# ACMEAtronOmatic/DSen2

Hardware: AMD Instinct MI355X
Metric: 32x32x6 patches/sec (DSen2_20, d=6, batch 512) (higher is better)
Workload: dtype f32; 1 GPU; DSen2_20 d=6 F=128 fp32, 512 synthetic 32x32 patches (4+6 bands) per GPU per step, he_uniform random-init weights; batch_per_gpu=512, parallelism=patch-sharded dp1, backend=rccl, output_gather=False

## Files before the change

### dsen2_amd/DSen2Net.py

```python
import ctypes
import sys
import threading

import numpy as np
import torch

from . import _lib, weights as _weights

RES_SCALE = 0.1
PRECISIONS = {'fp32': 0, 'bf16': 1, 'bf16x3': 2}


def _ptr(t):
    return ctypes.c_void_p(t.data_ptr()) if t is not None else ctypes.c_void_p(0)


def _stream_ptr(device):
    return ctypes.c_void_p(torch.cuda.current_stream(device).cuda_stream)


class S2Model(object):

    def __init__(self, input_shape, num_layers, feature_size, device=None, precision='fp32'):
        if len(input_shape) not in (2, 3):
# ... 96 lines not shown

    def profile_forward(self, xs, out=None, iters=10, warm=3):
        n, _, h, w = xs[0].shape
        out = self._check_out(out, n, h, w)
        ws = self._get_workspace(self.workspace_bytes(n, h, w))
        ms = (ctypes.c_float * 5)()
        with torch.cuda.device(self.device):
            _lib.call('dsen2_model_forward_profile', self._handle, _ptr(xs[0]), _ptr(xs[1]),
                      _ptr(xs[2]) if len(xs) == 3 else ctypes.c_void_p(0), _ptr(out), n, h, w,
                      _ptr(ws), ws.numel(), _stream_ptr(self.device), int(warm), int(iters), ms)
        return dict(forward_ms=ms[0], first_ms=ms[1], body_ms=ms[2], out_ms=ms[3], wall_ms=ms[4])

    def body_launches(self, n, h, w):
        with torch.cuda.device(self.device):
            r = _lib.load().dsen2_model_body_launches(self._handle, int(n), int(h), int(w))
        if r < 0:
            raise _lib.DSen2Error(r, _lib.load().dsen2_last_error().decode())
        return r

    def batch_limit(self, h, w):
        per = self.workspace_bytes(1, h, w)
        return max(1, int(self.max_workspace_bytes // per))

    def preferred_batch(self, h, w):
        limit = self.batch_limit(h, w)
        if self.precision == 'fp32' or self.num_layers <= 0:
            return limit
        cus = int(torch.cuda.get_device_properties(self.device).multi_processor_count)
        n = (limit // cus) * cus
        while n >= cus:
# ... 339 lines not shown
    xb = to_blocked(x_bf16)
    out = None
    if epilogue == 0:
        out = torch.empty((n, feat // 8, h, w, 8), dtype=torch.bfloat16, device=x_bf16.device)
    elif epilogue == 3:
        out = torch.empty((n, h, w, feat), dtype=torch.float32, device=x_bf16.device)
    with torch.cuda.device(x_bf16.device):
        _lib.call('dsen2_conv3x3_body_bf16', _ptr(xb), kernel_hwio.ctypes.data_as(_lib.c_float_p),
                  bias.ctypes.data_as(_lib.c_float_p), _ptr(res_hi), _ptr(res_lo), _ptr(out), n, h, w, feat, int(epilogue),
                  float(res_scale), _stream_ptr(x_bf16.device))
    if epilogue == 1:
        return res_hi, res_lo
    return from_blocked(out) if epilogue == 0 else out


def conv3x3_nhwc(x, kernel_hwio, bias, epilogue=0, aux=None, res_scale=RES_SCALE, ref=False):
    n, h, w, cin = x.shape
    kernel_hwio = np.ascontiguousarray(kernel_hwio, np.float32)
    bias = np.ascontiguousarray(bias, np.float32)
    cout = kernel_hwio.shape[3]
    if epilogue == 2:
        out = torch.empty((n, cout, h, w), dtype=torch.float32, device=x.device)
    else:
        out = torch.empty((n, h, w, cout), dtype=torch.float32, device=x.device)
    with torch.cuda.device(x.device):
        _lib.call('dsen2_conv3x3_nhwc_ref' if ref else 'dsen2_conv3x3_nhwc', _ptr(x), kernel_hwio.ctypes.data_as(_lib.c_float_p),
                  bias.ctypes.data_as(_lib.c_float_p), _ptr(aux), _ptr(out), n, h, w, cin, cout, int(epilogue),
                  float(res_scale), _stream_ptr(x.device))
    return out
```

### dsen2_amd/_lib.py

```python
import ctypes
import os
import sys

_HERE = os.path.dirname(os.path.abspath(__file__))
LIB_PATH = os.environ.get('DSEN2_HIP_LIB') or os.path.join(_HERE, 'libdsen2_hip.so')

OK = 0
ERR_INVALID, ERR_HIP, ERR_NO_WEIGHTS, ERR_WORKSPACE, ERR_NO_DEVICE, ERR_NOMEM, ERR_INTERNAL = -1, -2, -3, -4, -5, -6, -7
DTYPE_U16, DTYPE_F32 = 0, 1
DTYPE_F64 = 2

c_float_p = ctypes.POINTER(ctypes.c_float)
c_int_p = ctypes.POINTER(ctypes.c_int)
c_void_p = ctypes.c_void_p
c_int = ctypes.c_int
c_size_t = ctypes.c_size_t

SIGNATURES = {
    'dsen2_version': (ctypes.c_char_p, []),
    'dsen2_last_error': (ctypes.c_char_p, []),
    'dsen2_device_count': (c_int, []),
    'dsen2_model_create': (c_int, [ctypes.POINTER(c_void_p), c_int, c_int, c_int, c_int, c_int, c_int]),
    'dsen2_model_destroy': (None, [c_void_p]),
    'dsen2_model_num_params': (c_size_t, [c_void_p]),
    'dsen2_model_load_weights': (c_int, [c_void_p, c_float_p, c_size_t]),
    'dsen2_model_workspace_bytes': (c_int, [c_void_p, c_int, c_int, c_int, ctypes.POINTER(c_size_t)]),
    'dsen2_model_forward': (c_int, [c_void_p, c_void_p, c_void_p, c_void_p, c_void_p, c_int, c_int, c_int,
                                    c_void_p, c_size_t, c_void_p]),
    'dsen2_model_body_launches': (c_int, [c_void_p, c_int, c_int, c_int]),
    'dsen2_model_forward_timed': (c_int, [c_void_p, c_void_p, c_void_p, c_void_p, c_void_p, c_int, c_int, c_int,
                                          c_void_p, c_size_t, c_void_p, c_int, c_float_p]),
    'dsen2_model_forward_profile': (c_int, [c_void_p, c_void_p, c_void_p, c_void_p, c_void_p, c_int, c_int, c_int,
                                            c_void_p, c_size_t, c_void_p, c_int, c_int, c_float_p]),
    'dsen2_conv3x3_nhwc': (c_int, [c_void_p, c_float_p, c_float_p, c_void_p, c_void_p, c_int, c_int, c_int, c_int,
                                   c_int, c_int, ctypes.c_float, c_void_p]),
    'dsen2_conv3x3_nhwc_ref': (c_int, [c_void_p, c_float_p, c_float_p, c_void_p, c_void_p, c_int, c_int, c_int, c_int,
                                       c_int, c_int, ctypes.c_float, c_void_p]),
    'dsen2_split_f32': (c_int, [c_void_p, c_void_p, c_void_p, c_int, c_int, c_int, c_int, c_void_p]),
    'dsen2_join_f32': (c_int, [c_void_p, c_void_p, c_void_p, c_int, c_int, c_int, c_int, c_void_p]),
    'dsen2_conv3x3_body_bf16': (c_int, [c_void_p, c_float_p, c_float_p, c_void_p, c_void_p, c_void_p, c_int, c_int, c_int,
                                        c_int, c_int, ctypes.c_float, c_void_p]),
    'dsen2_conv3x3_first_planes': (c_int, [c_void_p, c_void_p, c_void_p, c_int, c_int, c_int, c_float_p, c_float_p, c_int, c_int,
                                           c_void_p, c_void_p, c_int, c_int, c_int, c_void_p]),
    'dsen2_split3_f32': (c_int, [c_void_p, c_void_p, c_void_p, c_int, c_int, c_int, c_int, c_void_p]),
    'dsen2_conv3x3_body_bf16x3': (c_int, [c_void_p, c_float_p, c_float_p, c_void_p, c_void_p, c_void_p, c_int, c_int, c_int,
                                          c_int, c_int, ctypes.c_float, c_void_p]),
    'dsen2_model_time_body_conv': (c_int, [c_void_p, c_int, c_void_p, c_void_p, c_void_p, c_int, c_int, c_int, c_int,
                                           c_void_p, c_float_p]),
    'dsen2_model_train_workspace_bytes': (c_int, [c_void_p, c_int, c_int, c_int, ctypes.POINTER(c_size_t)]),
    'dsen2_model_gradients': (c_int, [c_void_p, c_void_p, c_void_p, c_void_p, c_void_p, c_void_p, c_void_p, c_void_p, c_int,
                                      c_int, c_int, c_void_p, c_size_t, c_void_p]),
    'dsen2_model_get_weights': (c_int, [c_void_p, c_void_p, c_void_p]),
# ... 75 lines not shown
```

### dsen2_amd/build.py

```python
import concurrent.futures
import os
import subprocess
import sys
import tempfile

HERE = os.path.dirname(os.path.abspath(__file__))
CSRC = os.path.join(HERE, 'csrc')
SOURCES = ['conv3x3_body32.hip', 'conv3x3_body16w.hip', 'conv3x3_out.hip', 'conv3x3_out_mfma.hip', 'conv3x3_mfma.hip', 'conv3x3_first.hip', 'conv3x3_first16.hip', 'patch_ops.hip', 'down_pixel_aggr.hip', 'imresize.hip', 'conv_plan.hip', 'capi.hip',
           'conv3x3_wgrad.hip', 'train_ops.hip', 'capi_train.hip']
HEADERS = [os.path.join(CSRC, "dsen2_internal.h"), os.path.join(CSRC, "conv_plan.h"), os.path.join(CSRC, "capi_internal.h"), os.path.join(CSRC, "conv3x3_dma.h"), os.path.join(CSRC, "conv3x3_bf16_common.h"), os.path.join(os.path.dirname(HERE), 'include', 'dsen2_hip.h')]
LIB = os.path.join(HERE, 'libdsen2_hip.so')
DIAG_LIB = os.path.join(os.path.dirname(HERE), 'build', 'libdsen2_hip_diag.so')
HIPCC = os.environ.get('HIPCC', '/opt/rocm/bin/hipcc')
FLAGS = ['--offload-arch=gfx950', '-O3', '-std=c++17', '-fPIC', '-fno-gpu-rdc', '-ffp-contract=off',
         '-Wall', '-Wno-unused-function', '-Werror=array-bounds']
JOBS = int(os.environ.get('DSEN2_BUILD_JOBS', '4'))


def needs_build(lib=LIB):
    if not os.path.exists(lib):
        return True
    t = os.path.getmtime(lib)
    deps = [os.path.join(CSRC, s) for s in SOURCES] + HEADERS + [os.path.abspath(__file__),
                                                                os.path.join(HERE, 'asm_contract.py')]
# ... 41 lines not shown
```

### dsen2_amd/csrc/capi.hip

```cpp

#include <chrono>
#include <cstdarg>
#include <cstdio>
#include <cstring>
#include <exception>
#include <new>
#include <vector>

#include "capi_internal.h"

using namespace dsen2;

namespace {

thread_local char g_err[512] = "";

#ifdef DSEN2_DIAG
Tuning g_diag_tuning;
unsigned long long* g_diag_stamps = nullptr;
#endif
Tuning default_tuning() {
#ifdef DSEN2_DIAG
  return g_diag_tuning;
#else
// ... 94 lines not shown
    return p;
  };
  r.x0 = take(align_up(pix * 16));
  r.a = take(full);
  if (m->precision == 1) {
    r.hi = take(half); r.lo = take(half); r.tbf = take(half);
  } else if (m->precision == 2) {
    r.hx = take(full); r.lo16 = take(half); r.t2 = take(full);
  } else {
    r.t = take(full);
  }
  r.bytes = off * sizeof(float);
  return r;
}

int forward_launches(const dsen2_model* m, const float* x10, const float* x20, const float* x60, float* out, int n, int h, int w,
                     const ForwardWs& B, size_t keep_step, bool x0_packed, hipStream_t stream, const hipEvent_t* ev) {
  const float* P = m->dev_params;
  const int d = m->num_layers;
  if (ev) HIP_TRY(hipEventRecord(ev[0], stream));
  if (int rc = first_layer(m, x10, x20, x60, n, h, w, B, x0_packed, stream)) return rc;
  if (ev) HIP_TRY(hipEventRecord(ev[1], stream));
  if (m->precision == 2 && d > 0) {
    if (int rc = body16(m, B.hx, B.lo16, B.t2, B.a, n, h, w, stream)) return rc;
  } else if (m->precision == 1 && d > 0) {
    if (int rc = body16(m, B.hi, B.lo, B.tbf, B.a, n, h, w, stream)) return rc;
  } else {
    for (int l = 1; l <= d; ++l) {
      const Layer& LA = m->layers[2 * l - 1];
      const Layer& LB = m->layers[2 * l];
      const float* x_in = B.a + (size_t)(l - 1) * keep_step;
      float* t = B.t + (size_t)(l - 1) * keep_step;
      HIP_TRY(launch(LA.plan, make_params(x_in, LA.weights(P), LA.bias(P), nullptr, t, n, h, w, 0, 0.f), LA.plan.epilogue, m->tune, stream));
      HIP_TRY(launch(LB.plan, make_params(t, LB.weights(P), LB.bias(P), x_in, B.a + (size_t)l * keep_step, n, h, w, 0, 0.1f),
                     LB.plan.epilogue, m->tune, stream));
    }
  }
  if (ev) HIP_TRY(hipEventRecord(ev[2], stream));
  {
    const Layer& L = m->layers.back();
    const float* skip = m->c60 > 0 ? x60 : x20;
// ... 50 lines not shown
    HIP_TRY(hipEventElapsedTime(&v, e[1], e[2])); sum[2] += v;
    HIP_TRY(hipEventElapsedTime(&v, e[2], e[3])); sum[3] += v;
  }
  for (int k = 0; k < 4; ++k) ms[k] = (float)(sum[k] / iters);
  double wall = std::chrono::duration<double, std::milli>(t1 - t0).count();
  if (warm > 0) {
    float span = 0.f;
    HIP_TRY(hipEventElapsedTime(&span, evs.ev.front(), evs.ev.back()));
    wall = span;
  }
  ms[4] = (float)(wall / iters);
  return DSEN2_OK;
}

static int conv3x3_nhwc(const float* dev_in, const float* host_kernel, const float* host_bias, const float* dev_aux, float* dev_out,
                        int n, int h, int w, int cin, int cout, int epilogue, float res_scale, void* stream_, const Tuning& tune) {
  if (!dev_in || !host_kernel || !host_bias || !dev_out) return fail(DSEN2_ERR_INVALID, "NULL argument");
  if (epilogue != kEpiRelu && epilogue != kEpiResidual && epilogue != kEpiSkipNCHW) return fail(DSEN2_ERR_INVALID, "epilogue %d", epilogue);
  if (epilogue != kEpiRelu && !dev_aux) return fail(DSEN2_ERR_INVALID, "epilogue %d needs dev_aux", epilogue);
  if (int rc = check_shape(nullptr, n, h, w)) return rc;
  const ConvRole role = epilogue == kEpiSkipNCHW ? ConvRole::Output
                        : cin <= 16 ? (epilogue == kEpiRelu ? ConvRole::First : ConvRole::DgradOutput)
                        : epilogue == kEpiRelu ? ConvRole::BodyA : ConvRole::BodyB;
  ConvPlan pl;
  if (!plan_conv(role, cin, cout, 0, tune, nullptr, &pl) || pl.cin_pad != cin)
    return fail(DSEN2_ERR_INVALID, "unsupported conv %d->%d epilogue %d", cin, cout, epilogue);
  hipStream_t stream = (hipStream_t)stream_;
  std::vector<float> staged(pl.floats);
  pack(pl, host_kernel, host_bias, staged.data());
  return launch_once_with_temp("conv3x3", staged.data(), staged.size() * sizeof(float), stream, [&](char* dev) {
    const float* wpk = reinterpret_cast<const float*>(dev);
    return launch(pl, make_params(dev_in, wpk, wpk + pl.bias_off, dev_aux, dev_out, n, h, w, cout, res_scale), epilogue, tune, stream);
  });
}

static int conv3x3_body16(int precision, const void* dev_in, const float* host_kernel, const float* host_bias, void* s0, void* s1,
                          void* dev_out, int n, int h, int w, int feat, int epilogue, float res_scale, void* stream_) {
  const bool x3 = precision == 2;
  if (!dev_in || !host_kernel || !host_bias) return fail(DSEN2_ERR_INVALID, "NULL argument");
  if (feat != 128 && feat != 256) return fail(DSEN2_ERR_INVALID, "feat %d unsupported", feat);
  if (epilogue != kEpiRelu && epilogue != kEpiResidual && epilogue != kEpiResidualF32) return fail(DSEN2_ERR_INVALID, "epilogue %d", epilogue);
  if (epilogue != kEpiRelu && (!s0 || !s1))
    return fail(DSEN2_ERR_INVALID, x3 ? "residual epilogue needs the stream's tensors" : "residual epilogue needs the hi and lo planes");
  if (epilogue != kEpiResidual && !dev_out) return fail(DSEN2_ERR_INVALID, "dev_out is NULL");
  if (int rc = check_shape(nullptr, n, h, w)) return rc;
  hipStream_t stream = (hipStream_t)stream_;
  const Tuning tune = default_tuning();
// ... 43 lines not shown

const char* dsen2_version(void) {
#ifdef DSEN2_DIAG
  return "dsen2_hip 0.3-diag (gfx950; fp32 MFMA 32x32x2 / bf16 MFMA 16x16x32 / bf16x3; DIAGNOSTIC build)";
#else
  return "dsen2_hip 0.3 (gfx950; fp32 MFMA 32x32x2 / bf16 MFMA 16x16x32 / bf16x3)";
#endif
}
const char* dsen2_last_error(void) { return g_err; }

#ifdef DSEN2_DIAG
int dsen2_diag_set(int key, int value) {
  Tuning& t = g_diag_tuning;
  switch (key) {
    case 0:
      if (value != 0 && (value < 11 || value > 14)) return fail(DSEN2_ERR_INVALID, "body variant %d unknown", value);
      t.first = value == 0 ? FirstKernel::Tile16 : FirstKernel::Direct;
      t.body = value == 0 ? BodyKernel::Tile : BodyKernel::Body32;
      t.body32 = value == 0 ? Body32Form::DeferStagger : static_cast<Body32Form>(value - 11);
      return DSEN2_OK;
    case 2:
      if (value != 0 && value != 2 && value != 3) return fail(DSEN2_ERR_INVALID, "output variant %d unknown", value);
      t.out = value == 2 ? OutKernel::MfmaThenValu : value == 3 ? OutKernel::Valu : OutKernel::Tile;
      return DSEN2_OK;
    case 1: t.ablate = value; return DSEN2_OK;
    case 3: t.grid_cap = value; return DSEN2_OK;
    case 4: t.chain = value; return DSEN2_OK;
    case 5: t.first_ablate = value; return DSEN2_OK;
    case 6: t.out_ablate = value; return DSEN2_OK;
  }
  return fail(DSEN2_ERR_INVALID, "unknown diagnostic key %d", key);
// ... 26 lines not shown
    if (c10 <= 0 || c20 <= 0 || c60 < 0 || num_layers < 0) return fail(DSEN2_ERR_INVALID, "bad channel/layer counts");
    if (feature_size != 128 && feature_size != 256)
      return fail(DSEN2_ERR_INVALID, "feature_size %d unsupported (128 or 256)", feature_size);
    if (precision < 0 || precision > 2)
      return fail(DSEN2_ERR_INVALID, "precision %d unknown (0 = fp32, 1 = bf16 operands, 2 = bf16x3)", precision);
    const int cin = c10 + c20 + c60;
    const int cout = c60 > 0 ? c60 : c20;
    if (cin > 16) return fail(DSEN2_ERR_INVALID, "%d input channels > 16", cin);
    if (cout > 32) return fail(DSEN2_ERR_INVALID, "%d output channels > 32", cout);
    dsen2_model* m = new (std::nothrow) dsen2_model();
    if (!m) return fail(DSEN2_ERR_INVALID, "out of host memory");
    m->c10 = c10; m->c20 = c20; m->c60 = c60; m->cin = cin; m->cout = cout;
    m->num_layers = num_layers; m->feat = feature_size; m->precision = precision;
    m->dev_params = nullptr; m->loaded = false; m->train = nullptr;
    m->tune = default_tuning();
    if (hipGetDevice(&m->device) != hipSuccess) {
      delete m;
      return fail(DSEN2_ERR_NO_DEVICE, "no HIP device");
    }
    if (!plan_network(c10, c20, c60, num_layers, feature_size, precision, m->tune, m)) {
      delete m;
      return fail(DSEN2_ERR_INVALID, "no kernel for a layer of this network");
    }
    *out = m;
    return DSEN2_OK;
  });
}

void dsen2_model_destroy(dsen2_model* m) {
  if (!m) return;
  train_state_destroy(m->train);
  if (m->dev_params) (void)hipFree(m->dev_params);
  delete m;
}

size_t dsen2_model_num_params(const dsen2_model* m) { return m ? m->n_params : 0; }

int dsen2_model_load_weights(dsen2_model* m, const float* host_flat, size_t count) {
  return guarded([&]() -> int {
    if (!m || !host_flat) return fail(DSEN2_ERR_INVALID, "NULL argument");
    if (count != m->n_params)
      return fail(DSEN2_ERR_INVALID, "expected %zu parameters, got %zu", m->n_params, count);
    if (int rc = check_device(m)) return rc;
    std::vector<float> staged(m->dev_param_floats);
    for (const Layer& L : m->layers) {
      const float* k = host_flat + L.flat_off;
// ... 18 lines not shown
  return guarded([&] { return forward(m, x10, x20, x60, out, n, h, w, workspace, workspace_bytes, stream, nullptr); });
}

int dsen2_model_body_launches(const dsen2_model* m, int n, int h, int w) {
  return guarded([&]() -> int {
    if (!m) return fail(DSEN2_ERR_INVALID, "NULL model");
    if (int rc = check_shape(m, n, h, w)) return rc;
    if (int rc = check_device(m)) return rc;
    int dev = 0, cus = 0;
    if (hipGetDevice(&dev) != hipSuccess || hipDeviceGetAttribute(&cus, hipDeviceAttributeMultiprocessorCount, dev) != hipSuccess)
      return fail(DSEN2_ERR_NO_DEVICE, "no HIP device");
    return may_chain(m) && body16w_chain_patches_per_wg(n, h, w, m->feat, cus) > 0 ? 1 : 2 * m->num_layers;
  });
}

int dsen2_model_forward_timed(dsen2_model* m, const float* x10, const float* x20, const float* x60, float* out, int n, int h, int w,
                              void* workspace, size_t workspace_bytes, void* stream, int iters, float* body_ms_per_launch) {
  return guarded([&]() -> int {
    if (!body_ms_per_launch) return fail(DSEN2_ERR_INVALID, "NULL result");
    if (!m || m->num_layers <= 0) return fail(DSEN2_ERR_INVALID, "model has no residual blocks");
    float ms[5];
    int rc = forward_profile(m, x10, x20, x60, out, n, h, w, workspace, workspace_bytes, stream, 0, iters, ms);
    if (rc == DSEN2_OK) *body_ms_per_launch = ms[2] / (2.0f * m->num_layers);
    return rc;
  });
}

int dsen2_model_forward_profile(dsen2_model* m, const float* x10, const float* x20, const float* x60, float* out, int n, int h,
                                int w, void* workspace, size_t workspace_bytes, void* stream, int warm, int iters, float* ms5) {
  return guarded([&] { return forward_profile(m, x10, x20, x60, out, n, h, w, workspace, workspace_bytes, stream, warm, iters, ms5); });
}

int dsen2_conv3x3_nhwc(const float* dev_in, const float* host_kernel, const float* host_bias, const float* dev_aux, float* dev_out,
                       int n, int h, int w, int cin, int cout, int epilogue, float res_scale, void* stream) {
  return guarded([&] {
    return conv3x3_nhwc(dev_in, host_kernel, host_bias, dev_aux, dev_out, n, h, w, cin, cout, epilogue, res_scale, stream, default_tuning());
  });
}

int dsen2_conv3x3_nhwc_ref(const float* dev_in, const float* host_kernel, const float* host_bias, const float* dev_aux,
                           float* dev_out, int n, int h, int w, int cin, int cout, int epilogue, float res_scale, void* stream) {
  return guarded([&] {
    return conv3x3_nhwc(dev_in, host_kernel, host_bias, dev_aux, dev_out, n, h, w, cin, cout, epilogue, res_scale, stream,
                        Tuning::reference());
  });
}

int dsen2_split_f32(const float* dev_in, void* dev_hi, void* dev_lo, int n, int h, int w, int c, void* stream) {
  return guarded([&]() -> int {
    if (int rc = check_split_args(dev_in, dev_hi, dev_lo, n, h, w, c)) return rc;
    if (n == 0) return DSEN2_OK;
// ... 139 lines not shown
```

### dsen2_amd/csrc/capi_internal.h

```cpp
#pragma once
#include <exception>
#include <new>
#include <vector>

#include "../../include/dsen2_hip.h"
#include "conv_plan.h"

namespace dsen2 {

int fail(int code, const char* fmt, ...);

#define HIP_TRY(expr)                                                                                              \
  do {                                                                                                             \
    hipError_t e_ = (expr);                                                                                        \
    if (e_ != hipSuccess) return dsen2::fail(DSEN2_ERR_HIP, "%s failed: %s", #expr, hipGetErrorString(e_));   \
  } while (0)

template <class F>
int guarded(F&& body) noexcept {
  try {
    return body();
  } catch (const std::bad_alloc&) {
    return fail(DSEN2_ERR_NOMEM, "out of host memory");
  } catch (const std::exception& e) {
// ... 4 lines not shown
}

struct TrainState;
void train_state_destroy(TrainState* t);
int train_state_after_load(dsen2_model* m);

}

struct dsen2_model : dsen2::NetworkPlan {
  int c10, c20, c60, cin, cout, num_layers, feat, precision;
  int device;
  dsen2::Tuning tune;
  float* dev_params;
  bool loaded;
  dsen2::TrainState* train;
};

namespace dsen2 {

inline int check_shape(const dsen2_model* m, int n, int h, int w) {
  if (n <= 0 || h <= 0 || w <= 0) return fail(DSEN2_ERR_INVALID, "bad shape n=%d h=%d w=%d", n, h, w);
  if ((size_t)h * w * (size_t)(m ? m->feat : 256) >= ((size_t)1 << 29))
    return fail(DSEN2_ERR_INVALID, "one image of %dx%d exceeds 2^31 activation bytes", h, w);
  return DSEN2_OK;
}

inline int check_device(const dsen2_model* m) {
  int dev = -1;
  if (hipGetDevice(&dev) != hipSuccess) return fail(DSEN2_ERR_NO_DEVICE, "no HIP device");
  if (dev != m->device)
// ... 42 lines not shown
  if (e != hipSuccess) return fail(DSEN2_ERR_HIP, "%s launch: %s", what, hipGetErrorString(e));
  return DSEN2_OK;
}

struct ForwardWs {
  float* x0 = nullptr;
  float* a = nullptr;
  float* t = nullptr;
  void *hi = nullptr, *lo = nullptr, *tbf = nullptr;
  void *hx = nullptr, *lo16 = nullptr, *t2 = nullptr;
  size_t bytes = 0;
};
ForwardWs forward_ws(const dsen2_model* m, int n, int h, int w, char* base);
int forward_launches(const dsen2_model* m, const float* x10, const float* x20, const float* x60, float* out, int n, int h, int w,
                     const ForwardWs& B, size_t keep_step, bool x0_packed, hipStream_t stream, const hipEvent_t* ev);

}
```

### dsen2_amd/csrc/conv3x3_body32.hip

```cpp
#include <type_traits>

#include "conv3x3_dma.h"

namespace dsen2 {

namespace {

typedef float f32x4 __attribute__((ext_vector_type(4)));
typedef float f32x16 __attribute__((ext_vector_type(16)));
typedef unsigned u32x4 __attribute__((ext_vector_type(4)));

using dma::KC; using dma::NT; using dma::THREADS; using dma::QS; using dma::IN_BYTES; using dma::IN_BLOCKS;
using dma::WCH; using dma::NWBUF; using dma::LDS_BYTES; using dma::wait_vmcnt;
constexpr int KSTEPS = 4;
constexpr int PB = 2, MB = 2;
static_assert((8 * kHalo) % 16 == 0, "rows R and R+8 of a pixel block sit on the same banks");

}

template <int CIN, int COUT, int EPI, int ABL, int PRE, bool STG, bool DEFER>
__global__ __launch_bounds__(THREADS, 2) void conv3x3_body32_kernel(const ConvParams p, const int n_items) {
  constexpr int NCC = CIN / KC;
  constexpr int NS = COUT / NT;
  static_assert(NCC % 2 == 0, "input double buffer parity");
// ... 255 lines not shown
  auto kern = conv3x3_body32_kernel<CIN, COUT, EPI, ABL, PRE, STG, DEFER>;
  static KernelOnce once;
  int cus = 0;
  hipError_t e = once.prepare(reinterpret_cast<const void*>(kern), LDS_BYTES, &cus);
  if (e != hipSuccess) return e;
  const long long items = (long long)p.n * p.tiles_x * p.tiles_y * (COUT / NT);
  if (items <= 0 || items > 0x7fffffffLL) return hipErrorInvalidValue;
  const int grid = (int)(items < cus ? items : cus);
  hipLaunchKernelGGL(kern, dim3(grid), dim3(THREADS), LDS_BYTES, stream, p, (int)items);
  return hipGetLastError();
}

template <int F>
static hipError_t launch_body32_feat(const ConvParams& p, int epilogue, Body32Form form, hipStream_t stream) {
  const bool relu = epilogue == kEpiRelu;
#ifdef DSEN2_DIAG
  if (form == Body32Form::Plain || form == Body32Form::StaggerA) {
    if (!relu) return launch_body32_one<F, F, kEpiResidual, 0, 2, false>(p, stream);
    return form == Body32Form::Plain ? launch_body32_one<F, F, kEpiRelu, 0, 0, false>(p, stream) : launch_body32_one<F, F, kEpiRelu, 0, 0, true>(p, stream);
  }
  if (form == Body32Form::DeferStaggerA && !relu) return launch_body32_one<F, F, kEpiResidual, 0, 0, false, true>(p, stream);
#else
  if (form != Body32Form::DeferStagger) return hipErrorInvalidValue;
#endif
  return relu ? launch_body32_one<F, F, kEpiRelu, 0, 0, true, true>(p, stream) : launch_body32_one<F, F, kEpiResidual, 0, 0, true, true>(p, stream);
}

hipError_t launch_conv3x3_body32(const ConvParams& p, int feat, int epilogue, Body32Form form, int ablate, hipStream_t stream) {
  if ((size_t)p.h * p.w * feat * 4 >= 0x80000000ull) return hipErrorNotSupported;
#ifdef DSEN2_DIAG
// ... 18 lines not shown
```

### dsen2_amd/csrc/conv_plan.h

```cpp
#pragma once
#include <vector>

#include "dsen2_internal.h"

namespace dsen2 {

enum class ConvRole { First, BodyA, BodyB, Output, DgradBody, DgradOutput };
enum class ConvKernel {
  Tile,
  Body32,
  Body16,
  Body16x3,
  Out
};

constexpr size_t kAlignFloats = 64;
inline size_t align_up(size_t v) { return (v + kAlignFloats - 1) / kAlignFloats * kAlignFloats; }

struct ConvPlan {
  ConvRole role;
  ConvKernel kernel;
  int epilogue;
  int cin, cout;
  int cin_pad, cout_pad;
// ... 1 lines not shown
  int real_channels;
  Body32Form body32;
  bool out_mfma;
  bool first_direct;
  int first16_planes;
  size_t weight_floats, bias_off, first16_off, floats;
};

struct BandGroups { int c10, c20, c60; };
bool plan_conv(ConvRole role, int cin, int cout, int precision, const Tuning& tune, const BandGroups* bands, ConvPlan* plan);
void pack(const ConvPlan& plan, const float* kernel_hwio, const float* bias, float* dst);
hipError_t launch(const ConvPlan& plan, const ConvParams& p, int epilogue, const Tuning& tune, hipStream_t stream);

inline hipError_t try_launch(hipError_t e, bool* done) { *done = e == hipSuccess; return e == hipErrorNotSupported ? hipSuccess : e; }

struct Layer {
  ConvPlan plan;
  size_t off, flat_off;
  const float* weights(const float* params) const { return params + off; }
  const float* bias(const float* params) const { return params + off + plan.bias_off; }
  const float* first16(const float* params) const { return params + off + plan.first16_off; }
};
struct NetworkPlan {
  std::vector<Layer> layers;
  size_t n_params = 0;
  size_t dev_param_floats = 0;
  size_t chain_stride = 0;
};
bool plan_network(int c10, int c20, int c60, int num_layers, int feat, int precision, const Tuning& tune, NetworkPlan* net);

// ... 2 lines not shown
```

### dsen2_amd/csrc/conv_plan.hip

```cpp
#include <cstring>
#include <vector>

#include "conv_plan.h"

namespace dsen2 {

namespace {

constexpr int kBody16Chunk = 32;

bool sentinel2(const BandGroups* b) { return b && b->c10 == 4 && b->c20 == 6 && (b->c60 == 0 || b->c60 == 2); }

void pack_tile_weights(const float* k, const ConvPlan& pl, float* dst) {
  const int ncc = pl.cin_pad / pl.kc, nslab = pl.cout_pad / pl.nt, ng = pl.kc / 4;
  size_t i = 0;
  for (int slab = 0; slab < nslab; ++slab)
    for (int cc = 0; cc < ncc; ++cc)
      for (int tap = 0; tap < 9; ++tap)
        for (int gg = 0; gg < ng; ++gg)
          for (int o = 0; o < pl.nt; ++o)
            for (int j = 0; j < 4; ++j, ++i) {
              const int c = cc * pl.kc + 4 * gg + j, oc = slab * pl.nt + o;
              dst[i] = (c < pl.cin && oc < pl.cout) ? k[((size_t)tap * pl.cin + c) * pl.cout + oc] : 0.f;
            }
// ... 115 lines not shown
      const hipError_t e = pl.out_mfma ? try_launch(launch_conv3x3_out_mfma(pm, pl.cin_pad, stream, t.out_ablate), &done) : hipSuccess;
      return e != hipSuccess || done ? e : launch_conv3x3_out_valu(p, pl.cin_pad, stream);
    }
    case ConvKernel::Body32: return launch_conv3x3_body32(p, pl.cin_pad, epilogue, pl.body32, t.ablate, stream);
    case ConvKernel::Body16: return launch_conv3x3_body16w(p, pl.cin_pad, epilogue, false, t.ablate & 1023, stream, t.grid_cap);
    case ConvKernel::Body16x3: return launch_conv3x3_body16w(p, pl.cin_pad, epilogue, true, 0, stream);
    case ConvKernel::Tile: {
      const int mask = pl.role == ConvRole::Output ? t.out_ablate : pl.cin_pad == pl.cout_pad ? t.ablate : 0;
      if (mask != 0) return hipErrorInvalidValue;
      return launch_conv3x3_tile(p, pl.cin_pad, pl.cout_pad, epilogue, pl.real_channels, stream);
    }
  }
  return hipErrorInvalidValue;
}

bool plan_network(int c10, int c20, int c60, int num_layers, int feat, int precision, const Tuning& tune, NetworkPlan* net) {
  const BandGroups bands{c10, c20, c60};
  *net = NetworkPlan{};
  auto add = [&](ConvRole role, int ci, int co, int prec) {
    Layer L;
    if (!plan_conv(role, ci, co, prec, tune, &bands, &L.plan)) return false;
    L.flat_off = net->n_params;
    net->n_params += (size_t)9 * ci * co + co;
    L.off = net->dev_param_floats;
    net->dev_param_floats += L.plan.floats;
    net->layers.push_back(L);
    return true;
  };
  if (!add(ConvRole::First, c10 + c20 + c60, feat, num_layers > 0 ? precision : 0)) return false;
  for (int i = 0; i < num_layers; ++i)
// ... 8 lines not shown
```

### dsen2_amd/csrc/dsen2_internal.h

```cpp
#pragma once
#include <hip/hip_runtime.h>
#include <stddef.h>
#include <stdint.h>

#include <mutex>

namespace dsen2 {


constexpr int kTile = 16;
constexpr int kHalo = kTile + 2;
constexpr int kHaloPix = kHalo * kHalo;

enum Epilogue : int {
  kEpiRelu = 0, kEpiResidual = 1, kEpiSkipNCHW = 2,
  kEpiResidualF32 = 3,
  kEpiReluSplit = 4
};

struct ConvParams {
  const float* in;
  const float* wpk;
  const float* bias;
  const float* aux;
  float* out;
  void* out2;
  int n, h, w;
  int tiles_x, tiles_y;
  int cout_real;
  float res_scale;
  unsigned long long* diag;
};

enum class FirstKernel { Direct, Tile16 };
enum class BodyKernel { Body32, Tile };
enum class Body32Form { StaggerA, Plain, DeferStaggerA, DeferStagger };
enum class OutKernel { MfmaThenValu, Valu, Tile };
struct Tuning {
  FirstKernel first = FirstKernel::Direct;
  BodyKernel body = BodyKernel::Body32;
  Body32Form body32 = Body32Form::DeferStagger;
  OutKernel out = OutKernel::MfmaThenValu;
  int ablate = 0;
  int grid_cap = 0;
  int first_ablate = 0;
  int out_ablate = 0;
  int chain = 1;
  static Tuning reference() { Tuning t; t.first = FirstKernel::Tile16; t.body = BodyKernel::Tile; t.out = OutKernel::Tile; return t; }
};

struct KernelOnce {
// ... 20 lines not shown
  }
};

hipError_t launch_conv3x3_tile(const ConvParams& p, int cin_pad, int cout_pad, int epilogue, int real_channels, hipStream_t stream);
hipError_t launch_conv3x3_out_valu(const ConvParams& p, int feat, hipStream_t stream);
void pack_out_valu_weights_host(const float* kernel_hwio, int cin, int cout, float* dst);
hipError_t launch_conv3x3_out_mfma(const ConvParams& p, int feat, hipStream_t stream, int ablate = 0);
size_t out_mfma_weight_floats(int cin);
void pack_out_mfma_weights_host(const float* kernel_hwio, int cin, int cout, float* dst);
struct FirstInputs { const float* x60; int c10, c20, c60; };
hipError_t launch_conv3x3_first(const ConvParams& p, const FirstInputs& f, int cout, int epilogue, hipStream_t stream, int ablate = 0);
hipError_t launch_conv3x3_first16(const ConvParams& p, const FirstInputs& f, int cout, bool x3, hipStream_t stream);
size_t first16_weight_u16(int cout, bool x3);
void pack_first16_weights_host(const float* kernel_hwio, int cin, int cout, bool x3, uint16_t* dst);
hipError_t launch_conv3x3_body32(const ConvParams& p, int feat, int epilogue, Body32Form form, int ablate, hipStream_t stream);
hipError_t launch_conv3x3_body16w(const ConvParams& p, int feat, int epilogue, bool x3, int ablate, hipStream_t stream, int grid_cap = 0);
hipError_t launch_split3_f32(const float* in_nhwc, void* hx, void* lo, int n, int h, int w, int c, hipStream_t stream);
struct ChainArgs {
  void* hi;
  void* lo;
  void* t;
  float* out_f32;
  unsigned layer_stride;
  int n_layers;
  int patches_per_wg;
  int seamless;
};
hipError_t launch_conv3x3_body16w_chain(const ConvParams& p, const ChainArgs& c, int feat, hipStream_t stream, int ablate = 0,
                                        bool x3 = false);
int body16w_chain_patches_per_wg(int n, int h, int w, int feat, int cus);
// ... 32 lines not shown
```

### include/dsen2_hip.h

```cpp
#ifndef DSEN2_HIP_H
#define DSEN2_HIP_H

#include <stddef.h>

#ifdef __cplusplus
extern "C" {
#endif

#define DSEN2_OK 0
#define DSEN2_ERR_INVALID (-1)
#define DSEN2_ERR_HIP (-2)
#define DSEN2_ERR_NO_WEIGHTS (-3)
#define DSEN2_ERR_WORKSPACE (-4)
#define DSEN2_ERR_NO_DEVICE (-5)
#define DSEN2_ERR_NOMEM (-6)
#define DSEN2_ERR_INTERNAL (-7)

typedef struct dsen2_model dsen2_model;

const char *dsen2_version(void);
const char *dsen2_last_error(void);
int dsen2_device_count(void);

int dsen2_model_create(dsen2_model **out, int c10, int c20, int c60, int num_layers, int feature_size,
                       int precision);
void dsen2_model_destroy(dsen2_model *m);

size_t dsen2_model_num_params(const dsen2_model *m);

int dsen2_model_load_weights(dsen2_model *m, const float *host_flat, size_t count);

int dsen2_model_workspace_bytes(const dsen2_model *m, int n, int h, int w, size_t *bytes);

int dsen2_model_forward(dsen2_model *m, const float *dev_x10, const float *dev_x20, const float *dev_x60,
                        float *dev_out, int n, int h, int w, void *dev_workspace, size_t workspace_bytes,
                        void *stream);

int dsen2_model_body_launches(const dsen2_model *m, int n, int h, int w);

int dsen2_model_forward_timed(dsen2_model *m, const float *x10, const float *x20, const float *x60, float *out,
                              int n, int h, int w, void *workspace, size_t workspace_bytes, void *stream, int iters,
                              float *body_ms_per_launch);

int dsen2_model_forward_profile(dsen2_model *m, const float *x10, const float *x20, const float *x60, float *out,
                                int n, int h, int w, void *workspace, size_t workspace_bytes, void *stream, int warm,
                                int iters, float *ms5);

int dsen2_conv3x3_nhwc(const float *dev_in, const float *host_kernel, const float *host_bias,
                       const float *dev_aux, float *dev_out, int n, int h, int w, int cin, int cout,
                       int epilogue, float res_scale, void *stream);

int dsen2_conv3x3_nhwc_ref(const float *dev_in, const float *host_kernel, const float *host_bias,
                           const float *dev_aux, float *dev_out, int n, int h, int w, int cin, int cout,
                           int epilogue, float res_scale, void *stream);

int dsen2_split_f32(const float *dev_in_nhwc, void *dev_hi, void *dev_lo, int n, int h, int w, int c, void *stream);
int dsen2_join_f32(const void *dev_hi, const void *dev_lo, float *dev_out_nhwc, int n, int h, int w, int c, void *stream);

int dsen2_conv3x3_body_bf16(const void *dev_in_bf16, const float *host_kernel, const float *host_bias,
                            void *dev_res_hi, void *dev_res_lo, void *dev_out, int n, int h, int w, int feat,
                            int epilogue, float res_scale, void *stream);

int dsen2_split3_f32(const float *dev_in_nhwc, void *dev_hx, void *dev_lo, int n, int h, int w, int c, void *stream);
int dsen2_conv3x3_body_bf16x3(const void *dev_in_planes, const float *host_kernel, const float *host_bias,
                              void *dev_res_hx, void *dev_res_lo, void *dev_out, int n, int h, int w, int feat,
                              int epilogue, float res_scale, void *stream);

int dsen2_conv3x3_first_planes(const float *dev_x10, const float *dev_x20, const float *dev_x60, int c10, int c20, int c60,
                               const float *host_kernel, const float *host_bias, int feat, int precision,
// ... 51 lines not shown
```

Measured before the change: 40100 patches/s.

## Offload tail images to a concurrent vector-ALU conv kernel on a side stream

For fp32 models, the change splits the body's residual-block convolutions so a small share of images runs on a second stream. That share uses a new vector-ALU (FMA) conv kernel sized to fit in the LDS and register headroom left by the main matrix-core kernel. The main kernel, switched to a new 'Slim' form, handles the rest of the batch. The aim is to fill the partial last wave of workgroups and use idle VALU capacity alongside the matrix-core path. The cost is extra stream/event synchronisation per forward and the risk that the two kernels contend for CUs and slow the main path.

```diff
diff --git a/dsen2_amd/DSen2Net.py b/dsen2_amd/DSen2Net.py
--- a/dsen2_amd/DSen2Net.py
+++ b/dsen2_amd/DSen2Net.py
@@ -134,6 +134,16 @@
     def body_launches(self, n, h, w):
         with torch.cuda.device(self.device):
             r = _lib.load().dsen2_model_body_launches(self._handle, int(n), int(h), int(w))
+        if r < 0:
+            raise _lib.DSen2Error(r, _lib.load().dsen2_last_error().decode())
+        return r
+
+    def set_side_images(self, s):
+        _lib.call('dsen2_model_set_side_images', self._handle, int(s))
+
+    def side_images(self, n, h, w):
+        with torch.cuda.device(self.device):
+            r = _lib.load().dsen2_model_side_images(self._handle, int(n), int(h), int(w))
         if r < 0:
             raise _lib.DSen2Error(r, _lib.load().dsen2_last_error().decode())
         return r
@@ -503,17 +513,20 @@
     return from_blocked(out) if epilogue == 0 else out
 
 
-def conv3x3_nhwc(x, kernel_hwio, bias, epilogue=0, aux=None, res_scale=RES_SCALE, ref=False):
+def conv3x3_nhwc(x, kernel_hwio, bias, epilogue=0, aux=None, res_scale=RES_SCALE, ref=False, valu=False, out=None):
+    if ref and valu:
+        raise ValueError('ref and valu name two different kernels')
     n, h, w, cin = x.shape
     kernel_hwio = np.ascontiguousarray(kernel_hwio, np.float32)
     bias = np.ascontiguousarray(bias, np.float32)
     cout = kernel_hwio.shape[3]
-    if epilogue == 2:
-        out = torch.empty((n, cout, h, w), dtype=torch.float32, device=x.device)
-    else:
-        out = torch.empty((n, h, w, cout), dtype=torch.float32, device=x.device)
+    shape = (n, cout, h, w) if epilogue == 2 else (n, h, w, cout)
+    if out is None:
+        out = torch.empty(shape, dtype=torch.float32, device=x.device)
+    elif tuple(out.shape) != shape or out.dtype != torch.float32 or not out.is_contiguous() or out.device != x.device:
+        raise ValueError('out must be a contiguous float32 tensor of shape %r on %s' % (shape, x.device))
     with torch.cuda.device(x.device):
-        _lib.call('dsen2_conv3x3_nhwc_ref' if ref else 'dsen2_conv3x3_nhwc', _ptr(x), kernel_hwio.ctypes.data_as(_lib.c_float_p),
+        _lib.call('dsen2_conv3x3_nhwc_valu' if valu else 'dsen2_conv3x3_nhwc_ref' if ref else 'dsen2_conv3x3_nhwc', _ptr(x), kernel_hwio.ctypes.data_as(_lib.c_float_p),
                   bias.ctypes.data_as(_lib.c_float_p), _ptr(aux), _ptr(out), n, h, w, cin, cout, int(epilogue),
                   float(res_scale), _stream_ptr(x.device))
     return out
diff --git a/dsen2_amd/_lib.py b/dsen2_amd/_lib.py
--- a/dsen2_amd/_lib.py
+++ b/dsen2_amd/_lib.py
@@ -36,6 +36,10 @@
                                    c_int, c_int, ctypes.c_float, c_void_p]),
     'dsen2_conv3x3_nhwc_ref': (c_int, [c_void_p, c_float_p, c_float_p, c_void_p, c_void_p, c_int, c_int, c_int, c_int,
                                        c_int, c_int, ctypes.c_float, c_void_p]),
+    'dsen2_conv3x3_nhwc_valu': (c_int, [c_void_p, c_float_p, c_float_p, c_void_p, c_void_p, c_int, c_int, c_int, c_int,
+                                        c_int, c_int, ctypes.c_float, c_void_p]),
+    'dsen2_model_set_side_images': (c_int, [c_void_p, c_int]),
+    'dsen2_model_side_images': (c_int, [c_void_p, c_int, c_int, c_int]),
     'dsen2_split_f32': (c_int, [c_void_p, c_void_p, c_void_p, c_int, c_int, c_int, c_int, c_void_p]),
     'dsen2_join_f32': (c_int, [c_void_p, c_void_p, c_void_p, c_int, c_int, c_int, c_int, c_void_p]),
     'dsen2_conv3x3_body_bf16': (c_int, [c_void_p, c_float_p, c_float_p, c_void_p, c_void_p, c_void_p, c_int, c_int, c_int,
diff --git a/dsen2_amd/build.py b/dsen2_amd/build.py
--- a/dsen2_amd/build.py
+++ b/dsen2_amd/build.py
@@ -6,7 +6,7 @@
 
 HERE = os.path.dirname(os.path.abspath(__file__))
 CSRC = os.path.join(HERE, 'csrc')
-SOURCES = ['conv3x3_body32.hip', 'conv3x3_body16w.hip', 'conv3x3_out.hip', 'conv3x3_out_mfma.hip', 'conv3x3_mfma.hip', 'conv3x3_first.hip', 'conv3x3_first16.hip', 'patch_ops.hip', 'down_pixel_aggr.hip', 'imresize.hip', 'conv_plan.hip', 'capi.hip',
+SOURCES = ['conv3x3_body32.hip', 'conv3x3_body_valu.hip', 'conv3x3_body16w.hip', 'conv3x3_out.hip', 'conv3x3_out_mfma.hip', 'conv3x3_mfma.hip', 'conv3x3_first.hip', 'conv3x3_first16.hip', 'patch_ops.hip', 'down_pixel_aggr.hip', 'imresize.hip', 'conv_plan.hip', 'capi.hip',
            'conv3x3_wgrad.hip', 'train_ops.hip', 'capi_train.hip']
 HEADERS = [os.path.join(CSRC, "dsen2_internal.h"), os.path.join(CSRC, "conv_plan.h"), os.path.join(CSRC, "capi_internal.h"), os.path.join(CSRC, "conv3x3_dma.h"), os.path.join(CSRC, "conv3x3_bf16_common.h"), os.path.join(os.path.dirname(HERE), 'include', 'dsen2_hip.h')]
 LIB = os.path.join(HERE, 'libdsen2_hip.so')
diff --git a/dsen2_amd/csrc/capi.hip b/dsen2_amd/csrc/capi.hip
--- a/dsen2_amd/csrc/capi.hip
+++ b/dsen2_amd/csrc/capi.hip
@@ -132,10 +132,54 @@
   return r;
 }
 
+int side_images_for(const dsen2_model* m, int n, int h, int w) {
+  if (m->precision != 0 || m->num_layers <= 0 || m->tune.body != BodyKernel::Body32 || m->tune.ablate != 0) return 0;
+  if (m->side_images < 0 && m->tune.body32 != Body32Form::DeferStagger) return 0;
+  const int s = plan_side_images(n, h, w, m->feat, m->precision, m->num_layers, m->cus, m->side_images);
+  if (s >= n) return fail(DSEN2_ERR_INVALID, "side share of %d images needs a batch of more than %d (got %d)", s, s, n);
+  return s;
+}
+
+static int side_state(const dsen2_model* m) {
+  if (!m->side_stream) HIP_TRY(hipStreamCreateWithFlags(&m->side_stream, hipStreamNonBlocking));
+  if (!m->side_fork) HIP_TRY(hipEventCreateWithFlags(&m->side_fork, hipEventDisableTiming));
+  if (!m->side_join) HIP_TRY(hipEventCreateWithFlags(&m->side_join, hipEventDisableTiming));
+  return DSEN2_OK;
+}
+
+static int body32_split(const dsen2_model* m, int n, int h, int w, int s, const ForwardWs& B, size_t keep_step, hipStream_t stream) {
+  const float* P = m->dev_params;
+  const size_t skip = (size_t)(n - s) * h * w * m->feat;
+  std::lock_guard<std::mutex> lock(m->side_mu);
+  if (int rc = side_state(m)) return rc;
+  HIP_TRY(hipEventRecord(m->side_fork, stream));
+  HIP_TRY(hipStreamWaitEvent(m->side_stream, m->side_fork, 0));
+  for (int l = 1; l <= m->num_layers; ++l) {
+    const Layer& LA = m->layers[2 * l - 1];
+    const Layer& LB = m->layers[2 * l];
+    ConvPlan pa = LA.plan, pb = LB.plan;
+    pa.body32 = pb.body32 = Body32Form::Slim;
+    const float* x_in = B.a + (size_t)(l - 1) * keep_step;
+    float* t = B.t + (size_t)(l - 1) * keep_step;
+    float* x_out = B.a + (size_t)l * keep_step;
+    HIP_TRY(launch(pa, make_params(x_in, LA.weights(P), LA.bias(P), nullptr, t, n - s, h, w, 0, 0.f), pa.epilogue, m->tune, stream));
+    HIP_TRY(launch_conv3x3_body_valu(make_params(x_in + skip, LA.weights(P), LA.bias(P), nullptr, t + skip, s, h, w, 0, 0.f), m->feat,
+                                     pa.epilogue, m->side_stream));
+    HIP_TRY(launch(pb, make_params(t, LB.weights(P), LB.bias(P), x_in, x_out, n - s, h, w, 0, 0.1f), pb.epilogue, m->tune, stream));
+    HIP_TRY(launch_conv3x3_body_valu(make_params(t + skip, LB.weights(P), LB.bias(P), x_in + skip, x_out + skip, s, h, w, 0, 0.1f),
+                                     m->feat, pb.epilogue, m->side_stream));
+  }
+  HIP_TRY(hipEventRecord(m->side_join, m->side_stream));
+  HIP_TRY(hipStreamWaitEvent(stream, m->side_join, 0));
+  return DSEN2_OK;
+}
+
 int forward_launches(const dsen2_model* m, const float* x10, const float* x20, const float* x60, float* out, int n, int h, int w,
                      const ForwardWs& B, size_t keep_step, bool x0_packed, hipStream_t stream, const hipEvent_t* ev) {
   const float* P = m->dev_params;
   const int d = m->num_layers;
+  const int side = side_images_for(m, n, h, w);
+  if (side < 0) return side;
   if (ev) HIP_TRY(hipEventRecord(ev[0], stream));
   if (int rc = first_layer(m, x10, x20, x60, n, h, w, B, x0_packed, stream)) return rc;
   if (ev) HIP_TRY(hipEventRecord(ev[1], stream));
@@ -143,6 +187,8 @@
     if (int rc = body16(m, B.hx, B.lo16, B.t2, B.a, n, h, w, stream)) return rc;
   } else if (m->precision == 1 && d > 0) {
     if (int rc = body16(m, B.hi, B.lo, B.tbf, B.a, n, h, w, stream)) return rc;
+  } else if (side > 0) {
+    if (int rc = body32_split(m, n, h, w, side, B, keep_step, stream)) return rc;
   } else {
     for (int l = 1; l <= d; ++l) {
       const Layer& LA = m->layers[2 * l - 1];
@@ -223,7 +269,8 @@
 }
 
 static int conv3x3_nhwc(const float* dev_in, const float* host_kernel, const float* host_bias, const float* dev_aux, float* dev_out,
-                        int n, int h, int w, int cin, int cout, int epilogue, float res_scale, void* stream_, const Tuning& tune) {
+                        int n, int h, int w, int cin, int cout, int epilogue, float res_scale, void* stream_, const Tuning& tune,
+                        bool valu = false) {
   if (!dev_in || !host_kernel || !host_bias || !dev_out) return fail(DSEN2_ERR_INVALID, "NULL argument");
   if (epilogue != kEpiRelu && epilogue != kEpiResidual && epilogue != kEpiSkipNCHW) return fail(DSEN2_ERR_INVALID, "epilogue %d", epilogue);
   if (epilogue != kEpiRelu && !dev_aux) return fail(DSEN2_ERR_INVALID, "epilogue %d needs dev_aux", epilogue);
@@ -234,12 +281,14 @@
   ConvPlan pl;
   if (!plan_conv(role, cin, cout, 0, tune, nullptr, &pl) || pl.cin_pad != cin)
     return fail(DSEN2_ERR_INVALID, "unsupported conv %d->%d epilogue %d", cin, cout, epilogue);
+  if (valu && pl.kernel != ConvKernel::Body32) return fail(DSEN2_ERR_INVALID, "no vector-ALU kernel for conv %d->%d epilogue %d", cin, cout, epilogue);
   hipStream_t stream = (hipStream_t)stream_;
   std::vector<float> staged(pl.floats);
   pack(pl, host_kernel, host_bias, staged.data());
   return launch_once_with_temp("conv3x3", staged.data(), staged.size() * sizeof(float), stream, [&](char* dev) {
     const float* wpk = reinterpret_cast<const float*>(dev);
-    return launch(pl, make_params(dev_in, wpk, wpk + pl.bias_off, dev_aux, dev_out, n, h, w, cout, res_scale), epilogue, tune, stream);
+    const ConvParams p = make_params(dev_in, wpk, wpk + pl.bias_off, dev_aux, dev_out, n, h, w, cout, res_scale);
+    return valu ? launch_conv3x3_body_valu(p, pl.cin_pad, epilogue, stream) : launch(pl, p, epilogue, tune, stream);
   });
 }
 
@@ -313,7 +362,7 @@
   Tuning& t = g_diag_tuning;
   switch (key) {
     case 0:
-      if (value != 0 && (value < 11 || value > 14)) return fail(DSEN2_ERR_INVALID, "body variant %d unknown", value);
+      if (value != 0 && (value < 11 || value > 15)) return fail(DSEN2_ERR_INVALID, "body variant %d unknown", value);
       t.first = value == 0 ? FirstKernel::Tile16 : FirstKernel::Direct;
       t.body = value == 0 ? BodyKernel::Tile : BodyKernel::Body32;
       t.body32 = value == 0 ? Body32Form::DeferStagger : static_cast<Body32Form>(value - 11);
@@ -370,7 +419,7 @@
     m->num_layers = num_layers; m->feat = feature_size; m->precision = precision;
     m->dev_params = nullptr; m->loaded = false; m->train = nullptr;
     m->tune = default_tuning();
-    if (hipGetDevice(&m->device) != hipSuccess) {
+    if (hipGetDevice(&m->device) != hipSuccess || hipDeviceGetAttribute(&m->cus, hipDeviceAttributeMultiprocessorCount, m->device) != hipSuccess) {
       delete m;
       return fail(DSEN2_ERR_NO_DEVICE, "no HIP device");
     }
@@ -386,6 +435,9 @@
 void dsen2_model_destroy(dsen2_model* m) {
   if (!m) return;
   train_state_destroy(m->train);
+  if (m->side_fork) (void)hipEventDestroy(m->side_fork);
+  if (m->side_join) (void)hipEventDestroy(m->side_join);
+  if (m->side_stream) (void)hipStreamDestroy(m->side_stream);
   if (m->dev_params) (void)hipFree(m->dev_params);
   delete m;
 }
@@ -434,6 +486,21 @@
   });
 }
 
+int dsen2_model_set_side_images(dsen2_model* m, int s) {
+  if (!m || s < -1) return fail(DSEN2_ERR_INVALID, "bad argument");
+  if (s > 0 && (m->precision != 0 || m->num_layers <= 0)) return fail(DSEN2_ERR_INVALID, "only an fp32 model with residual blocks has a side share");
+  m->side_images = s;
+  return DSEN2_OK;
+}
+
+int dsen2_model_side_images(const dsen2_model* m, int n, int h, int w) {
+  return guarded([&]() -> int {
+    if (!m) return fail(DSEN2_ERR_INVALID, "NULL model");
+    if (int rc = check_shape(m, n, h, w)) return rc;
+    return side_images_for(m, n, h, w);
+  });
+}
+
 int dsen2_model_forward_timed(dsen2_model* m, const float* x10, const float* x20, const float* x60, float* out, int n, int h, int w,
                               void* workspace, size_t workspace_bytes, void* stream, int iters, float* body_ms_per_launch) {
   return guarded([&]() -> int {
@@ -455,6 +522,14 @@
                        int n, int h, int w, int cin, int cout, int epilogue, float res_scale, void* stream) {
   return guarded([&] {
     return conv3x3_nhwc(dev_in, host_kernel, host_bias, dev_aux, dev_out, n, h, w, cin, cout, epilogue, res_scale, stream, default_tuning());
+  });
+}
+
+int dsen2_conv3x3_nhwc_valu(const float* dev_in, const float* host_kernel, const float* host_bias, const float* dev_aux,
+                            float* dev_out, int n, int h, int w, int cin, int cout, int epilogue, float res_scale, void* stream) {
+  return guarded([&] {
+    return conv3x3_nhwc(dev_in, host_kernel, host_bias, dev_aux, dev_out, n, h, w, cin, cout, epilogue, res_scale, stream, default_tuning(),
+                        true);
   });
 }
 
diff --git a/dsen2_amd/csrc/capi_internal.h b/dsen2_amd/csrc/capi_internal.h
--- a/dsen2_amd/csrc/capi_internal.h
+++ b/dsen2_amd/csrc/capi_internal.h
@@ -1,5 +1,6 @@
 #pragma once
 #include <exception>
+#include <mutex>
 #include <new>
 #include <vector>
 
@@ -42,6 +43,11 @@
   float* dev_params;
   bool loaded;
   dsen2::TrainState* train;
+  int side_images = 0;
+  int cus = 0;
+  mutable std::mutex side_mu;
+  mutable hipStream_t side_stream = nullptr;
+  mutable hipEvent_t side_fork = nullptr, side_join = nullptr;
 };
 
 namespace dsen2 {
@@ -114,5 +120,6 @@
 ForwardWs forward_ws(const dsen2_model* m, int n, int h, int w, char* base);
 int forward_launches(const dsen2_model* m, const float* x10, const float* x20, const float* x60, float* out, int n, int h, int w,
                      const ForwardWs& B, size_t keep_step, bool x0_packed, hipStream_t stream, const hipEvent_t* ev);
+int side_images_for(const dsen2_model* m, int n, int h, int w);
 
 }
diff --git a/dsen2_amd/csrc/conv3x3_body32.hip b/dsen2_amd/csrc/conv3x3_body32.hip
--- a/dsen2_amd/csrc/conv3x3_body32.hip
+++ b/dsen2_amd/csrc/conv3x3_body32.hip
@@ -293,6 +293,8 @@
 template <int F>
 static hipError_t launch_body32_feat(const ConvParams& p, int epilogue, Body32Form form, hipStream_t stream) {
   const bool relu = epilogue == kEpiRelu;
+  if (form == Body32Form::Slim)
+    return relu ? launch_body32_one<F, F, kEpiRelu, 0, 0, false, false>(p, stream) : launch_body32_one<F, F, kEpiResidual, 0, 0, false, false>(p, stream);
 #ifdef DSEN2_DIAG
   if (form == Body32Form::Plain || form == Body32Form::StaggerA) {
     if (!relu) return launch_body32_one<F, F, kEpiResidual, 0, 2, false>(p, stream);
diff --git a/dsen2_amd/csrc/conv3x3_body_valu.hip b/dsen2_amd/csrc/conv3x3_body_valu.hip
--- /dev/null
+++ b/dsen2_amd/csrc/conv3x3_body_valu.hip
@@ -0,0 +1,132 @@
+#include "dsen2_internal.h"
+
+namespace dsen2 {
+
+namespace {
+
+typedef float f32x4 __attribute__((ext_vector_type(4)));
+typedef float f32x16 __attribute__((ext_vector_type(16)));
+typedef unsigned u32x4 __attribute__((ext_vector_type(4)));
+typedef __attribute__((address_space(4))) const f32x16 const_f32x16;
+typedef __attribute__((address_space(4))) const f32x4 const_f32x4;
+
+constexpr int VT = 256;
+constexpr int NT = 128;
+constexpr int KC = 32;
+constexpr int WCH = KC * NT;
+constexpr int kSideLds = 8192;
+static_assert(kSideLds > (163840 - 152576) / 2 && kSideLds <= 163840 - 152576, "LDS placement window");
+
+}
+
+template <int F, int EPI>
+__global__ __launch_bounds__(VT) __attribute__((amdgpu_waves_per_eu(2, 2))) void conv3x3_body_valu_kernel(const ConvParams p) {
+  constexpr int NCC = F / KC;
+  constexpr int NS = F / NT;
+  constexpr int STEPS = NCC * 9 * 4;
+
+  const int lane = threadIdx.x & 63;
+  const int wave = __builtin_amdgcn_readfirstlane(threadIdx.x >> 6);
+  const int tile = blockIdx.x / NS, slab = blockIdx.x - tile * NS;
+  const int tiles_per_img = p.tiles_x * p.tiles_y;
+  const int img = tile / tiles_per_img;
+  const int trem = tile - img * tiles_per_img;
+  const int tyi = trem / p.tiles_x;
+  const int y = tyi * kTile + 4 * wave + (lane >> 4);
+  const int x = (trem - tyi * p.tiles_x) * kTile + (lane & 15);
+  const size_t img_floats = (size_t)p.h * p.w * F;
+  const unsigned img_bytes = (unsigned)(img_floats * 4);
+
+  const auto in_rsrc = __builtin_amdgcn_make_buffer_rsrc(const_cast<float*>(p.in) + img * img_floats, 0, img_bytes, 0x00020000);
+  auto x_off = [&](int step) -> unsigned {
+    const int cc = step / 36, r = step - cc * 36;
+    const int tap = r >> 2, s = r & 3;
+    const int dy = tap / 3, dx = tap - dy * 3;
+    const int yy = y + dy - 1, xx = x + dx - 1;
+    const bool ok = (unsigned)yy < (unsigned)p.h && (unsigned)xx < (unsigned)p.w;
+    return ok ? (unsigned)(((yy * p.w + xx) * F + cc * KC + 8 * s) * 4) : 0x80000000u;
+  };
+  auto load_x = [&](f32x4 (&xv)[2], int step) {
+    const unsigned off = x_off(step);
+    xv[0] = __builtin_bit_cast(f32x4, __builtin_amdgcn_raw_buffer_load_b128(in_rsrc, off, 0, 0));
+    xv[1] = __builtin_bit_cast(f32x4, __builtin_amdgcn_raw_buffer_load_b128(in_rsrc, off, 16, 0));
+  };
+
+  const const_f32x16* const wk = reinterpret_cast<const const_f32x16*>(reinterpret_cast<uintptr_t>(p.wpk + (size_t)slab * NCC * 9 * WCH));
+
+  float acc[NT];
+#pragma unroll
+  for (int o = 0; o < NT; ++o) acc[o] = 0.f;
+
+  f32x4 xc[2], xn[2];
+  load_x(xc, 0);
+#pragma unroll 1
+  for (int step = 0; step < STEPS; ++step) {
+    load_x(xn, step + 1 < STEPS ? step + 1 : step);
+    const const_f32x16* const w0 = wk + (size_t)(step >> 2) * (WCH / 16) + (step & 3) * (2 * NT * 4 / 16);
+    const const_f32x16* const w1 = w0 + NT * 4 / 16;
+    f32x16 wa = w0[0], wb = w1[0];
+#pragma unroll
+    for (int b = 0; b < NT / 4; ++b) {
+      f32x16 na = wa, nb = wb;
+      if (b + 1 < NT / 4) {
+        na = w0[b + 1];
+        nb = w1[b + 1];
+      }
+      __builtin_amdgcn_sched_barrier(0);
+#pragma unroll
+      for (int o = 0; o < 4; ++o)
+#pragma unroll
+        for (int j = 0; j < 4; ++j) {
+          acc[4 * b + o] = __builtin_fmaf(wa[4 * o + j], xc[0][j], acc[4 * b + o]);
+          acc[4 * b + o] = __builtin_fmaf(wb[4 * o + j], xc[1][j], acc[4 * b + o]);
+        }
+      wa = na;
+      wb = nb;
+    }
+    xc[0] = xn[0];
+    xc[1] = xn[1];
+  }
+
+  const bool ok = y < p.h && x < p.w;
+  const unsigned pix_off = ok ? (unsigned)(((y * p.w + x) * F + slab * NT) * 4) : 0x80000000u;
+  const auto out_rsrc = __builtin_amdgcn_make_buffer_rsrc(p.out + img * img_floats, 0, img_bytes, 0x00020000);
+  const auto aux_rsrc = __builtin_amdgcn_make_buffer_rsrc(
+      const_cast<float*>(p.aux) + (EPI == kEpiResidual ? img * img_floats : 0), 0, EPI == kEpiResidual ? img_bytes : 0, 0x00020000);
+  const const_f32x4* const bk = reinterpret_cast<const const_f32x4*>(reinterpret_cast<uintptr_t>(p.bias + slab * NT));
+#pragma unroll
+  for (int b = 0; b < NT / 4; ++b) {
+    const f32x4 bias = bk[b];
+    f32x4 v = {acc[4 * b], acc[4 * b + 1], acc[4 * b + 2], acc[4 * b + 3]};
+    v = v + bias;
+    if constexpr (EPI == kEpiRelu) {
+#pragma unroll
+      for (int e = 0; e < 4; ++e) v[e] = fmaxf(v[e], 0.f);
+    } else {
+      const f32x4 rr = __builtin_bit_cast(f32x4, __builtin_amdgcn_raw_buffer_load_b128(aux_rsrc, pix_off, 16 * b, 0));
+      v = rr + v * p.res_scale;
+    }
+    __builtin_amdgcn_raw_buffer_store_b128(__builtin_bit_cast(u32x4, v), out_rsrc, pix_off, 16 * b, 0);
+  }
+}
+
+template <int F>
+static hipError_t launch_valu_feat(const ConvParams& p, int epilogue, hipStream_t stream) {
+  const long long wgs = (long long)p.n * p.tiles_x * p.tiles_y * (F / NT);
+  if (wgs <= 0 || wgs > 0x7fffffffLL) return hipErrorInvalidValue;
+  if (epilogue == kEpiRelu)
+    hipLaunchKernelGGL((conv3x3_body_valu_kernel<F, kEpiRelu>), dim3((unsigned)wgs), dim3(VT), kSideLds, stream, p);
+  else
+    hipLaunchKernelGGL((conv3x3_body_valu_kernel<F, kEpiResidual>), dim3((unsigned)wgs), dim3(VT), kSideLds, stream, p);
+  return hipGetLastError();
+}
+
+hipError_t launch_conv3x3_body_valu(const ConvParams& p, int feat, int epilogue, hipStream_t stream) {
+  if (epilogue != kEpiRelu && epilogue != kEpiResidual) return hipErrorInvalidValue;
+  if ((size_t)p.h * p.w * feat * 4 >= 0x80000000ull) return hipErrorNotSupported;
+  if (feat == 128) return launch_valu_feat<128>(p, epilogue, stream);
+  if (feat == 256) return launch_valu_feat<256>(p, epilogue, stream);
+  return hipErrorInvalidValue;
+}
+
+}
diff --git a/dsen2_amd/csrc/conv_plan.h b/dsen2_amd/csrc/conv_plan.h
--- a/dsen2_amd/csrc/conv_plan.h
+++ b/dsen2_amd/csrc/conv_plan.h
@@ -39,6 +39,8 @@
 
 inline hipError_t try_launch(hipError_t e, bool* done) { *done = e == hipSuccess; return e == hipErrorNotSupported ? hipSuccess : e; }
 
+int plan_side_images(int n, int h, int w, int feat, int precision, int num_layers, int cus, int requested);
+
 struct Layer {
   ConvPlan plan;
   size_t off, flat_off;
diff --git a/dsen2_amd/csrc/conv_plan.hip b/dsen2_amd/csrc/conv_plan.hip
--- a/dsen2_amd/csrc/conv_plan.hip
+++ b/dsen2_amd/csrc/conv_plan.hip
@@ -153,6 +153,16 @@
   return hipErrorInvalidValue;
 }
 
+int plan_side_images(int n, int h, int w, int feat, int precision, int num_layers, int cus, int requested) {
+  if (requested >= 0) return requested;
+  if (precision != 0 || feat != 128 || num_layers <= 0 || cus <= 0 || n <= 0) return 0;
+  const long long per = (long long)((h + kTile - 1) / kTile) * ((w + kTile - 1) / kTile) * (feat / 128);
+  const long long rounds = (n * per + cus - 1) / cus;
+  if (rounds < 2) return 0;
+  const long long s = n - (rounds - 1) * cus / per;
+  return s > 0 && s * 6 <= n ? (int)s : 0;
+}
+
 bool plan_network(int c10, int c20, int c60, int num_layers, int feat, int precision, const Tuning& tune, NetworkPlan* net) {
   const BandGroups bands{c10, c20, c60};
   *net = NetworkPlan{};
diff --git a/dsen2_amd/csrc/dsen2_internal.h b/dsen2_amd/csrc/dsen2_internal.h
--- a/dsen2_amd/csrc/dsen2_internal.h
+++ b/dsen2_amd/csrc/dsen2_internal.h
@@ -34,7 +34,7 @@
 
 enum class FirstKernel { Direct, Tile16 };
 enum class BodyKernel { Body32, Tile };
-enum class Body32Form { StaggerA, Plain, DeferStaggerA, DeferStagger };
+enum class Body32Form { StaggerA, Plain, DeferStaggerA, DeferStagger, Slim };
 enum class OutKernel { MfmaThenValu, Valu, Tile };
 struct Tuning {
   FirstKernel first = FirstKernel::Direct;
@@ -85,6 +85,7 @@
 size_t first16_weight_u16(int cout, bool x3);
 void pack_first16_weights_host(const float* kernel_hwio, int cin, int cout, bool x3, uint16_t* dst);
 hipError_t launch_conv3x3_body32(const ConvParams& p, int feat, int epilogue, Body32Form form, int ablate, hipStream_t stream);
+hipError_t launch_conv3x3_body_valu(const ConvParams& p, int feat, int epilogue, hipStream_t stream);
 hipError_t launch_conv3x3_body16w(const ConvParams& p, int feat, int epilogue, bool x3, int ablate, hipStream_t stream, int grid_cap = 0);
 hipError_t launch_split3_f32(const float* in_nhwc, void* hx, void* lo, int n, int h, int w, int c, hipStream_t stream);
 struct ChainArgs {
diff --git a/include/dsen2_hip.h b/include/dsen2_hip.h
--- a/include/dsen2_hip.h
+++ b/include/dsen2_hip.h
@@ -38,6 +38,9 @@
 
 int dsen2_model_body_launches(const dsen2_model *m, int n, int h, int w);
 
+int dsen2_model_set_side_images(dsen2_model *m, int s);
+int dsen2_model_side_images(const dsen2_model *m, int n, int h, int w);
+
 int dsen2_model_forward_timed(dsen2_model *m, const float *x10, const float *x20, const float *x60, float *out,
                               int n, int h, int w, void *workspace, size_t workspace_bytes, void *stream, int iters,
                               float *body_ms_per_launch);
@@ -53,6 +56,10 @@
 int dsen2_conv3x3_nhwc_ref(const float *dev_in, const float *host_kernel, const float *host_bias,
                            const float *dev_aux, float *dev_out, int n, int h, int w, int cin, int cout,
                            int epilogue, float res_scale, void *stream);
+
+int dsen2_conv3x3_nhwc_valu(const float *dev_in, const float *host_kernel, const float *host_bias,
+                            const float *dev_aux, float *dev_out, int n, int h, int w, int cin, int cout,
+                            int epilogue, float res_scale, void *stream);
 
 int dsen2_split_f32(const float *dev_in_nhwc, void *dev_hi, void *dev_lo, int n, int h, int w, int c, void *stream);
 int dsen2_join_f32(const void *dev_hi, const void *dev_lo, float *dev_out_nhwc, int n, int h, int w, int c, void *stream);
```

Result: no change. 39950 patches/s (-0.4%).
